# buq2/camera_calibrator

Hardware: AMD Instinct MI355X
Metric: LM residuals/sec (2*N_obs per LM iteration), single-camera intrinsics BA (higher is better)
Workload: dtype f64; 1 GPU; BASELINE.json configs[2]: single-camera intrinsics, 1000 frames x 500 pts per GPU, radial-tangential distortion, Zhang init, reference solver options (calibrator.cpp:314-321); frames_total=1000, points_per_frame=500, observations_total=500000, parallelism=frame-sharded x1, exchange=none

## Files before the change

camera_calibrator_amd/csrc/cc_device.hpp:

```cpp
#pragma once
#include "cc_common.hpp"

namespace cc {

typedef double d4 __attribute__((ext_vector_type(4)));
typedef double d2 __attribute__((ext_vector_type(2)));

constexpr int kStageDoublesPerWave = 64 * 16;

__device__ __forceinline__ int tri(int i, int j) { return i * (i + 1) / 2 + j; }

template <int CTRL>
__device__ __forceinline__ double dpp_f64(double v) {
  const int lo = __builtin_amdgcn_update_dpp(0, __double2loint(v), CTRL, 0xf, 0xf, false);
  const int hi = __builtin_amdgcn_update_dpp(0, __double2hiint(v), CTRL, 0xf, 0xf, false);
  return __hiloint2double(hi, lo);
}
__device__ __forceinline__ double row_pair_sum(double v) {
  const auto l = __builtin_amdgcn_permlane16_swap((unsigned)__double2loint(v), (unsigned)__double2loint(v), false, false);
  const auto h = __builtin_amdgcn_permlane16_swap((unsigned)__double2hiint(v), (unsigned)__double2hiint(v), false, false);
  return __hiloint2double((int)h[0], (int)l[0]) + __hiloint2double((int)h[1], (int)l[1]);
}
__device__ __forceinline__ double half_pair_sum(double v) {
  const auto l = __builtin_amdgcn_permlane32_swap((unsigned)__double2loint(v), (unsigned)__double2loint(v), false, false);
  const auto h = __builtin_amdgcn_permlane32_swap((unsigned)__double2hiint(v), (unsigned)__double2hiint(v), false, false);
  return __hiloint2double((int)h[0], (int)l[0]) + __hiloint2double((int)h[1], (int)l[1]);
}
template <int LOG2 = 0>
__device__ __forceinline__ double wave_sum_mod(double v) {
  static_assert(LOG2 >= 0 && LOG2 <= 3, "strides 1, 2, 4, 8");
  if (LOG2 == 0) v += dpp_f64<0xB1>(v);
  if (LOG2 <= 1) v += dpp_f64<0x4E>(v);
  if (LOG2 <= 2) v += dpp_f64<0x124>(v);
  v += dpp_f64<0x128>(v);
  return half_pair_sum(row_pair_sum(v));
}
__device__ __forceinline__ double wave_sum(double v) { return wave_sum_mod<0>(v); }
__device__ __forceinline__ double row16_sum(double v) {
  v += dpp_f64<0xB1>(v);
  v += dpp_f64<0x4E>(v);
  v += dpp_f64<0x141>(v);
  v += dpp_f64<0x140>(v);
  return v;
}
__device__ __forceinline__ double row16_max(double v) {
  v = fmax(v, dpp_f64<0xB1>(v));
  v = fmax(v, dpp_f64<0x4E>(v));
  v = fmax(v, dpp_f64<0x141>(v));
  v = fmax(v, dpp_f64<0x140>(v));
  return v;
}

__device__ __forceinline__ double lane_bcast(double v, int l) {
  return __hiloint2double(__builtin_amdgcn_readlane(__double2hiint(v), l), __builtin_amdgcn_readlane(__double2loint(v), l));
}

template <int S>
__device__ __forceinline__ bool chol_solve_rows(double (&a)[S], double b, double (&x)[S]) {
  bool ok = true;
  double inv[S];
#pragma unroll
  for (int j = 0; j < S; ++j) {
    const double d = lane_bcast(a[j], j);
    ok = ok && (d > 0.0) && isfinite(d);
    const double r = rsqrt(d);
    inv[j] = r;
    a[j] *= r;
#pragma unroll
    for (int k = j + 1; k < S; ++k) a[k] = fma(-a[j], lane_bcast(a[j], k), a[k]);
  }
#pragma unroll
  for (int j = 0; j < S; ++j) {
    const double y = lane_bcast(b, j) * inv[j];
    x[j] = y;
    b = fma(-a[j], y, b);
  }
#pragma unroll
  for (int i = S - 1; i >= 0; --i) {
    double acc = x[i];
#pragma unroll
    for (int k = i + 1; k < S; ++k) acc = fma(-lane_bcast(a[i], k), x[k], acc);
    x[i] = acc * inv[i];
  }
  return ok;
}

__device__ __forceinline__ void lds_barrier() { asm volatile("s_waitcnt lgkmcnt(0)\n\ts_barrier" ::: "memory"); }

__device__ __forceinline__ void wave_lds_fence() { __builtin_amdgcn_fence(__ATOMIC_ACQ_REL, "wavefront"); }

__device__ __forceinline__ void stage_row(double* stage, int lane, const double* v) {
#pragma unroll
  for (int j = 0; j < 8; ++j) {
    d2 val;
    val.x = v[2 * j];
    val.y = v[2 * j + 1];
    *reinterpret_cast<d2*>(&stage[lane * 16 + ((j ^ (lane & 7)) << 1)]) = val;
  }
}

__device__ __forceinline__ void gram_rows(const double* stage, int lane, d4& acc0, d4& acc1) {
  const int c = lane & 15, sub = lane >> 4;
#pragma unroll
  for (int m = 0; m < 16; m += 2) {
    const int r0 = 4 * m + sub, r1 = 4 * (m + 1) + sub;
    const double a0 = stage[r0 * 16 + (((c >> 1) ^ (r0 & 7)) << 1) + (c & 1)];
    const double a1 = stage[r1 * 16 + (((c >> 1) ^ (r1 & 7)) << 1) + (c & 1)];
    acc0 = __builtin_amdgcn_mfma_f64_16x16x4f64(a0, a0, acc0, 0, 0, 0);
    acc1 = __builtin_amdgcn_mfma_f64_16x16x4f64(a1, a1, acc1, 0, 0, 0);
  }
}

__device__ __forceinline__ void gram_operands(const double* stage, int lane, double* a) {
  const int c = lane & 15, sub = lane >> 4;
#pragma unroll
  for (int m = 0; m < 16; ++m) {
    const int r = 4 * m + sub;
    a[m] = stage[r * 16 + (((c >> 1) ^ (r & 7)) << 1) + (c & 1)];
  }
}

__device__ __forceinline__ void gram_products(const double* a, d4& acc0, d4& acc1) {
#pragma unroll
  for (int m = 0; m < 16; m += 2) {
    acc0 = __builtin_amdgcn_mfma_f64_16x16x4f64(a[m], a[m], acc0, 0, 0, 0);
    acc1 = __builtin_amdgcn_mfma_f64_16x16x4f64(a[m + 1], a[m + 1], acc1, 0, 0, 0);
  }
}

__device__ __forceinline__ void gram_rows_ahead(const double* stage, int lane, d4& acc0, d4& acc1) {
  double a[16];
  gram_operands(stage, lane, a);
  __builtin_amdgcn_sched_barrier(0);
  gram_products(a, acc0, acc1);
  __builtin_amdgcn_sched_barrier(0);
}



__device__ __forceinline__ int p2p_slot(const P2pDev& X, int kind, unsigned long long epoch, int rank) {
  const int base = kind == 0 ? 0 : 2 * kP2pMaxRanks * X.sw[0];
  return base + ((int)(epoch & 1ull) * kP2pMaxRanks + rank) * X.sw[kind];
}

__device__ inline void p2p_post(const P2pDev& X, int kind, unsigned long long epoch, int rank, int nranks,
                                const double* src, int n, int first = 0) {
  const int off = p2p_slot(X, kind, epoch, rank) + 2 * first;
  const unsigned long long tag = (epoch & 0xffffffffull) << 32;
  const int words = 2 * n;
  for (int idx = threadIdx.x; idx < words * nranks; idx += blockDim.x) {
    const int r = idx / words, w = idx - r * words;
    const unsigned long long bits = (unsigned long long)__double_as_longlong(src[w >> 1]);
    const unsigned long long half = (w & 1) ? (bits >> 32) : (bits & 0xffffffffull);
    __hip_atomic_store(X.box[r] + off + w, tag | half, __ATOMIC_RELAXED, __HIP_MEMORY_SCOPE_SYSTEM);
  }
}

__device__ __forceinline__ double p2p_poll_sum(const P2pDev& X, int kind, unsigned long long epoch, int rank, int nranks,
                                               int i, long long t0, int* s_ok) {
  const unsigned long long tag = epoch & 0xffffffffull;
  const unsigned long long* base = X.box[rank] + 2 * i;
  unsigned long long lo[kP2pMaxRanks], hi[kP2pMaxRanks];
  for (;;) {
    bool all = true;
#pragma unroll
    for (int r = 0; r < kP2pMaxRanks; ++r) {
      if (r < nranks) {
        const unsigned long long* p = base + p2p_slot(X, kind, epoch, r);
        lo[r] = __hip_atomic_load(p, __ATOMIC_RELAXED, __HIP_MEMORY_SCOPE_SYSTEM);
        hi[r] = __hip_atomic_load(p + 1, __ATOMIC_RELAXED, __HIP_MEMORY_SCOPE_SYSTEM);
      }
    }
#pragma unroll
    for (int r = 0; r < kP2pMaxRanks; ++r)
      if (r < nranks) all = all && (lo[r] >> 32) == tag && (hi[r] >> 32) == tag;
    if (all) break;
    if (wall_clock64() - t0 > kP2pTimeoutTicks) { *s_ok = 0; break; }
    __builtin_amdgcn_s_sleep(1);
  }
  double a = 0.0;
#pragma unroll
  for (int r = 0; r < kP2pMaxRanks; ++r)
    if (r < nranks) {
      const double v = __longlong_as_double((long long)((hi[r] << 32) | (lo[r] & 0xffffffffull)));
      a = r == 0 ? v : a + v;
    }
  return a;
}

__device__ inline double p2p_collect(const P2pDev& X, int kind, unsigned long long epoch, int rank, int nranks,
                                     int n, int* s_ok) {
  if (threadIdx.x == 0) *s_ok = 1;
  __syncthreads();
  double a = 0.0;
  if ((int)threadIdx.x < n) a = p2p_poll_sum(X, kind, epoch, rank, nranks, threadIdx.x, wall_clock64(), s_ok);
  __syncthreads();
  return a;
}

__device__ inline void p2p_collect_to(const P2pDev& X, int kind, unsigned long long epoch, int rank, int nranks,
                                      int n, double* dst, int* s_ok) {
  if (threadIdx.x == 0) *s_ok = 1;
  __syncthreads();
  const long long t0 = wall_clock64();
  for (int i = threadIdx.x; i < n; i += blockDim.x) dst[i] = p2p_poll_sum(X, kind, epoch, rank, nranks, i, t0, s_ok);
  __syncthreads();
}

}
```

camera_calibrator_amd/csrc/cc_intrinsics_persist.hip:

```cpp
#include "cc_intrinsics_persist.hpp"
#include "cc_persist_dev.hpp"
#include "cc_persist_pack.hpp"
#include "cc_persist_publish.hpp"
#include "cc_persist_sum.hpp"

namespace cc {


constexpr int persist_lds_doubles(int teams) { return teams * 4 * kStageDoublesPerWave + teams * 2 * 256 + teams * 192 + 512; }

enum { TM_Y = 0, TM_POSE = 60, TM_SP = 76, TM_STEP = 84, TM_R = 100, TM_T = 109, TM_KC = 112, TM_STEP2 = 122, TM_XN2 = 123,
       TM_QW = 124, TM_STAT = 128  };
enum { WG_INTR = 0 , WG_X = 64 , WG_DS = 66 ,
       WG_SS = 80 , WG_R0 = 96 ,
       WG_RO = 97 , WG_OPT = 100 ,
       WG_TAB = 104 ,
       WG_TGI = 416 , WG_TZ = 456  };

static_assert(TM_POSE - TM_Y >= 6 * 10 && TM_SP - TM_POSE >= 2 * 8 && TM_STEP - TM_SP >= 6 && TM_R - TM_STEP >= 15 && TM_T - TM_R >= 9 && TM_KC - TM_T >= 3 &&
              TM_STEP2 - TM_KC >= 9 && TM_QW - TM_XN2 >= 1 && TM_STAT - TM_QW >= 4 && TM_STAT + 4 + 9 <= 192,
              "per-team scratch: Y (6 x 10), two poses, pose scale, step (9 + 6), R, t, intrinsics, scalars, statistics row -- inside the 192 doubles persist_lds_doubles gives a team");
static_assert(WG_X - WG_INTR >= 2 * 16 && WG_DS - WG_X >= 2 && WG_SS - WG_DS >= 9 && WG_R0 - WG_SS >= 9 && WG_RO - WG_R0 >= 1 && WG_OPT - WG_RO >= 1 && WG_TAB - WG_OPT >= 4 &&
              WG_TZ - WG_TGI >= 80 / 2 && WG_TZ + 80 / 2 <= 512,
              "workgroup scratch: both intrinsics, broadcast (2 + 9), scales, options, tables of the 80-slot row -- inside the 512 doubles of persist_lds_doubles");

template <int NC, int NG, int BATCH = 8>
__device__ __forceinline__ void gather_rows(const u64* box, int G, unsigned tag, int ncols, int maxcol, double* s_part,
                                            double* out, unsigned* fail, int* s_ok, int tshift) {
  const int tid = threadIdx.x, col = tid % NC, grp = tid / NC;
  if (tid == 0) *s_ok = 1;
  __syncthreads();
  if (grp < NG && col < ncols) {
    double acc = 0.0;
    bool good = true;
    const long long t0 = wall_clock64();
    for (int r0 = grp; r0 < G && good; r0 += BATCH * NG) {
      u64 lo[BATCH], hi[BATCH];
      for (unsigned spins = 0;; ++spins) {
#pragma unroll
        for (int u = 0; u < BATCH; ++u) {
          const int r = r0 + u * NG;
          const u64* p = box + (size_t)(r < G ? r : r0) * (2 * NC) + 2 * col;
          lo[u] = ag_ld(p);
          hi[u] = ag_ld(p + 1);
        }
        bool ok = true;
#pragma unroll
        for (int u = 0; u < BATCH; ++u) ok = ok && (unsigned)(lo[u] >> 32) == tag && (unsigned)(hi[u] >> 32) == tag;
        if (ok) break;
        if ((spins & 63u) == 63u && (timed_out(t0, tshift) || ag_ld32(fail) != 0u)) { good = false; break; }
        __builtin_amdgcn_s_sleep(1);
      }
      if (!good) break;
#pragma unroll
      for (int u = 0; u < BATCH; ++u) {
        if (r0 + u * NG < G) {
          const double v = ungranule(lo[u], hi[u]);
          acc = col == maxcol ? fmax(acc, v) : acc + v;
        }
      }
    }
    s_part[grp * NC + col] = acc;
    if (!good) *s_ok = 0;
  }
  __syncthreads();
  if (tid < ncols) {
    double a = 0.0;
    if (tid == maxcol) { for (int g = 0; g < NG; ++g) a = fmax(a, s_part[g * NC + tid]); }
    else { for (int g = 0; g < NG; ++g) a += s_part[g * NC + tid]; }
    out[tid] = a;
  }
  __syncthreads();
}

template <int THREADS>
__device__ __forceinline__ void gather_stats4(const u64* box, int G, unsigned tag, double* s_part, double* out, unsigned* fail, int* s_ok, int tshift) {
  constexpr int RPT = 1024 / THREADS;
  static_assert(THREADS / 4 * RPT == kPMaxWorkers, "one statistics row per four threads: the host caps the worker grid at kPMaxWorkers");
  const int tid = threadIdx.x, col = tid & 3, lane = tid & 63, wave = tid >> 6;
  if (tid == 0) *s_ok = 1;
  __syncthreads();
  u64 lo[RPT], hi[RPT];
  bool good = true;
  const long long t0 = wall_clock64();
  for (unsigned spins = 0;; ++spins) {
    bool ok = true;
#pragma unroll
    for (int k = 0; k < RPT; ++k) {
      const int r = (tid >> 2) + k * (THREADS / 4);
      const u64* p = box + (size_t)(r < G ? r : 0) * (2 * kPStatCols) + 2 * col;
      lo[k] = ag_ld(p);
      hi[k] = ag_ld(p + 1);
    }
#pragma unroll
    for (int k = 0; k < RPT; ++k) ok = ok && (unsigned)(lo[k] >> 32) == tag && (unsigned)(hi[k] >> 32) == tag;
    if (ok) break;
    if ((spins & 63u) == 63u && (timed_out(t0, tshift) || ag_ld32(fail) != 0u)) { good = false; break; }
    __builtin_amdgcn_s_sleep(1);
  }
  double acc = 0.0;
#pragma unroll
  for (int k = 0; k < RPT; ++k)
    if ((tid >> 2) + k * (THREADS / 4) < G) acc += ungranule(lo[k], hi[k]);
  acc = wave_sum_mod<2>(acc);
  if (lane < 4) s_part[wave * 4 + lane] = acc;
  if (!good) *s_ok = 0;
  __syncthreads();
  if (tid < 4) {
    double a = 0.0;
#pragma unroll
    for (int w = 0; w < THREADS / 64; ++w) a += s_part[w * 4 + tid];
    out[tid] = a;
  }
  __syncthreads();
}

__device__ __forceinline__ size_t persist_box_word(int c, int g, int G) {
  return kPBoxColumnMajor ? ((size_t)c * (size_t)G + (size_t)g) * 2 : ((size_t)g * kPartialCols + (size_t)c) * 2;
}

template <int NG>
__device__ __forceinline__ void own_columns(const u64* box, u64* obox, int G, int w, unsigned tag, double* vals, unsigned* fail, int tid0, int tshift) {
  constexpr int kPer = (kPMaxWorkers + 63) / 64;
  int lane = tid0 & 63;
  asm volatile("" : "+v"(lane));
  asm volatile("" : "+s"(G));
  const int nc = (kPartialCols - 1 - w) / G + 1, items = nc * G, nL = persist_sum_groups(G);
  const u64* p[kPer];
#pragma unroll
  for (int u = 0; u < kPer; ++u) {
    const int i = lane + 64 * u, ic = i < items ? i : 0, k = ic / G;
    p[u] = box + persist_box_word(w + k * G, ic - k * G, G);
  }
  int gv[2], gn[2], gm[2];
#pragma unroll
  for (int u = 0; u < 2; ++u) {
    const int t = lane + 64 * u, tc = t < nc * nL ? t : 0, k = tc / nL, j = tc - k * nL;
    gv[u] = k * G + j * kPSumRows;
    gn[u] = persist_sum_group_rows(G, j);
    gm[u] = w + k * G == PC_GMAXP;
  }
  asm volatile("" : "+v"(gv[0]), "+v"(gv[1]), "+v"(gn[0]), "+v"(gn[1]), "+v"(gm[0]), "+v"(gm[1]));
  u64 lo[kPer], hi[kPer];
  bool good = true;
  const long long t0 = wall_clock64();
  for (unsigned spins = 0;; ++spins) {
#pragma unroll
    for (int u = 0; u < kPer; ++u) {
      lo[u] = ag_ld(p[u]);
      hi[u] = ag_ld(p[u] + 1);
    }
    bool ok = true;
#pragma unroll
    for (int u = 0; u < kPer; ++u) ok = ok && (unsigned)(lo[u] >> 32) == tag && (unsigned)(hi[u] >> 32) == tag;
    if (ok) break;
    if ((spins & 63u) == 63u && (timed_out(t0, tshift) || ag_ld32(fail) != 0u)) { good = false; break; }
    __builtin_amdgcn_s_sleep(1);
  }
  if (__any(!good)) {
    if (lane == 0) __hip_atomic_store(fail, 1u, __ATOMIC_RELAXED, __HIP_MEMORY_SCOPE_AGENT);
    return;
  }
#pragma unroll
  for (int u = 0; u < kPer; ++u)
    if (lane + 64 * u < items) vals[lane + 64 * u] = ungranule(lo[u], hi[u]);
  wave_lds_fence();
  double* Ls = vals + kPMaxWorkers + kPSumRows;
#pragma unroll
  for (int u = 0; u < 2; ++u)
    if (lane + 64 * u < nc * nL) Ls[lane + 64 * u] = persist_sum_group<NG>(vals + gv[u], gn[u], gm[u] != 0);
  wave_lds_fence();
  for (int k = lane; k < nc; k += 64) {
    const int c = w + k * G;
    const double total = persist_sum_group<NG>(Ls + k * nL, nL, c == PC_GMAXP);
    ag_st(obox + 2 * c, granule(tag, total, 0));
    ag_st(obox + 2 * c + 1, granule(tag, total, 1));
  }
}

__device__ __forceinline__ void gather_totals(const u64* box, unsigned tag, double* out, unsigned* fail, int* s_ok, int tshift) {
  const int tid = threadIdx.x;
  if (tid == 0) *s_ok = 1;
  __syncthreads();
  if (tid < kPartialCols) {
    const u64* p = box + 2 * tid;
    u64 lo, hi;
    bool good = true;
    const long long t0 = wall_clock64();
    for (unsigned spins = 0;; ++spins) {
      lo = ag_ld(p);
      hi = ag_ld(p + 1);
      if ((unsigned)(lo >> 32) == tag && (unsigned)(hi >> 32) == tag) break;
      if ((spins & 63u) == 63u && (timed_out(t0, tshift) || ag_ld32(fail) != 0u)) { good = false; break; }
      __builtin_amdgcn_s_sleep(1);
    }
    out[tid] = ungranule(lo, hi);
    if (!good) *s_ok = 0;
  }
  __syncthreads();
}

template <int THREADS>
__device__ __forceinline__ void persist_control(const IntrDev& P, const PersistDev& Q, double* lds) {
  double* s_part = lds;
  double* sv = lds + 1024;
  double* s_tot = lds + 1152;
  double* s_bc = lds + 1168;
  double* s_intr = lds + 1184;
  double* s_ss = lds + 1216;
  LmCtl* s_ctl = reinterpret_cast<LmCtl*>(lds + 1232);
  LmOpts* s_opts = reinterpret_cast<LmOpts*>(lds + 1252);
  cc_iteration* s_log = reinterpret_cast<cc_iteration*>(lds + 1264);
  int* s_int = reinterpret_cast<int*>(lds + 1296);
  u64* s_seq = reinterpret_cast<u64*>(lds + 1300);
  double* s_ccprev = lds + 1301;
  const int tid = threadIdx.x, wave = tid >> 6;
  static_assert(sizeof(cc_iteration) <= 32 * 8, "log record scratch");
  if (tid < (int)(sizeof(LmCtl) / 8)) reinterpret_cast<double*>(s_ctl)[tid] = 0.0;
  if (tid >= 32 && tid < 32 + (int)(sizeof(LmOpts) / 8)) reinterpret_cast<u64*>(s_opts)[tid - 32] = reinterpret_cast<const u64*>(P.opts)[tid - 32];
  if (tid >= 64 && tid < 64 + 32) s_intr[tid - 64] = 0.0;
  if (tid == 48 && P.host_pub) *s_seq = *P.pub_seq + 1ull;
  __syncthreads();
  if (tid < 9) s_intr[tid] = (Q.restart ? P.init_intr : P.intr)[tid];
  if (tid == 0) { s_int[1] = 0; s_int[3] = 0; s_int[5] = 0; s_int[6] = 0; s_int[7] = 0; *s_ccprev = 0.0; }
  __syncthreads();
  const LmOpts& o = *s_opts;
  const uint32_t mask = P.mask;

  for (int round = 0; round < Q.max_rounds; ++round) {
    const unsigned e1 = Q.epoch0 + 3u * (unsigned)round + 1u, e2 = e1 + 1u, e3 = e1 + 2u;
    const bool phase0 = round == 0;
    if (phase0) gather_rows<kPStatCols, THREADS / kPStatCols>(Q.sbox, Q.G, e1, 13, -1, s_part, s_tot, Q.fail, s_int, (phase0 ? Q.first_shift : Q.timeout_shift));
    else gather_stats4<THREADS>(Q.sbox, Q.G, e1, s_part, s_tot, Q.fail, s_int, (phase0 ? Q.first_shift : Q.timeout_shift));
    if (P.x.on) {
      const bool need = phase0 || (s_ctl->cand_pending && s_ctl->step_valid);
      if (need) {
        if (tid >= 13 && tid < 16) s_tot[tid] = 0.0;
        __syncthreads();
        const unsigned long long epoch = P.x.seq[1] + 1ull;
        p2p_post(P.x, 1, epoch, P.rank, P.nranks, s_tot, 16);
        int* s_ok2 = s_int + 4;
        const double a = p2p_collect(P.x, 1, epoch, P.rank, P.nranks, 16, s_ok2);
        if (tid < 16) s_tot[tid] = a;
        if (tid == 0) { P.x.seq[1] = epoch; if (!*s_ok2) s_int[0] = 0; }
        __syncthreads();
      }
    }
    if (tid == 0) {
      LmCtl c = *s_ctl;
      const int len0 = c.log_len, prev_cur = c.cur & 1, was_valid = c.step_valid;
      const int ro_now = s_int[3];
      const double prev_radius = c.radius;
      const double* kc0 = s_intr + (c.cur ? 16 : 0);
      const double* kc1 = s_intr + (c.cur ? 0 : 16);
      if (!s_int[0]) {
        __hip_atomic_store(Q.fail, 1u, __ATOMIC_RELAXED, __HIP_MEMORY_SCOPE_AGENT);
        c.done = 1; c.term = CC_FAILURE_EXCHANGE;
      } else if (phase0) {
        double xn2 = s_tot[ST_XNORM2];
#pragma unroll
        for (int i = 0; i < 9; ++i) {
          const double ki = kc0[i];
          xn2 += ki * ki;
          s_ss[i] = o.jacobi_scaling ? 1.0 / (1.0 + sqrt(s_tot[4 + i])) : 1.0;
        }
        lm_init(c, o, s_tot[ST_COST], sqrt(xn2));
      } else if (c.cand_pending) {
        double step2 = s_tot[ST_STEP2], xn2 = s_tot[ST_XNORM2];
        if (c.step_valid) {
#pragma unroll
          for (int i = 0; i < 9; ++i) {
            const double kc = kc1[i], k0 = kc0[i];
            const double d = kc - k0;
            step2 += d * d;
            xn2 += kc * kc;
          }
        }
        lm_decide(c, o, s_log, s_tot[ST_COST], s_tot[ST_QMODEL], step2, xn2);
      }
      if (!c.done && round + 1 >= Q.max_rounds) { c.done = 1; c.term = CC_NO_CONVERGENCE; }
      *s_ctl = c;
      s_int[1] = c.log_len != len0;
      s_int[2] = phase0 ? (!c.done && c.radius == o.initial_radius)
                        : (!ro_now && was_valid && !c.done && (c.cur & 1) == (prev_cur ^ 1) && c.radius == persist_spec_radius(prev_radius, o.max_radius));
      const bool accepted = !phase0 && (c.cur & 1) != prev_cur;
      if (ro_now) {
        s_int[6]++;
        if (!c.done) {
          if (Q.final_sweep == 1) s_int[5] = 1;
          if (accepted) s_int[7]++;
        }
      }
      int pred = 0;
      if (!c.done && s_int[0] && Q.final_sweep != 0 && !s_int[5] && !P.x.on && (phase0 || accepted)) {
        const double cc_k = phase0 ? 0.0 : s_log->cost_change;
        pred = Q.final_sweep == 2 || c.iter + 1 >= o.max_iterations || persist_predicts_end(cc_k, *s_ccprev, o.function_tolerance, c.x_cost);
      }
      if (accepted) *s_ccprev = s_log->cost_change;
      s_int[3] = pred;
      s_bc[0] = (double)((c.done ? 1 : 0) | ((c.cur & 1) << 3));
      s_bc[1] = c.radius;
#pragma unroll
      for (int i = 0; i < 9; ++i) s_bc[2 + i] = 0.0;
    }
    __syncthreads();
    const bool hit = s_int[2] != 0;
    const int pred_flag = s_int[3] ? 32 : 0;
    if (s_ctl->done || !hit) {
      if (tid < 22) ag_st(Q.xbox + tid, granule(e2, s_bc[tid >> 1], tid & 1));
      if (s_ctl->done) break;
    }
    const unsigned erow = hit ? e2 : e3;
    gather_totals(Q.lbox, erow, sv, Q.fail, s_int, (phase0 ? Q.first_shift : Q.timeout_shift));
    if (P.x.on) {
      if (tid >= kPartialCols && tid < kVecSolve) sv[tid] = 0.0;
      __syncthreads();
      if (tid == 0) { sv[kPartialCols + P.rank] = sv[PC_GMAXP]; sv[PC_GMAXP] = 0.0; }
      __syncthreads();
      const unsigned long long epoch = P.x.seq[0] + 1ull;
      p2p_post(P.x, 0, epoch, P.rank, P.nranks, sv, kVecSolve);
      int* s_ok2 = s_int + 4;
      const double a = p2p_collect(P.x, 0, epoch, P.rank, P.nranks, kVecSolve, s_ok2);
      if (tid < kVecSolve) sv[tid] = a;
      if (tid == 0) { P.x.seq[0] = epoch; if (!*s_ok2) s_int[0] = 0; }
      __syncthreads();
      if (tid == 0) {
        double g = 0.0;
        for (int r = 0; r < P.nranks && r < 32; ++r) g = fmax(g, sv[kPartialCols + r]);
        sv[PC_GMAXP] = g;
      }
      __syncthreads();
    }
    if (wave == 0) {
      int lane = tid & 63;
      asm volatile("" : "+v"(lane));
      const int cur = s_ctl->cur & 1;
      const double radius = s_ctl->radius;
      const double gl = (lane < 9 && !((mask >> lane) & 1u)) ? fabs(sv[PC_GS + lane]) : sv[PC_GMAXP];
      const double k_l = s_intr[cur * 16 + (lane < 9 ? lane : 8)], ss_l = s_ss[lane < 9 ? lane : 8];
      bool ok = !(sv[PC_FAIL] > 0.0);
      double x[9];
      {
#pragma clang fp contract(off)
        const int i = lane < 9 ? lane : 8;
        const bool pin_i = (mask >> i) & 1u;
        const double si = s_ss[i];
        const double damp = clampd(sv[PC_HDIAG + i] * (si * si), o.min_lm_diagonal, o.max_lm_diagonal) / radius;
        double a[9];
#pragma unroll
        for (int k = 0; k < 9; ++k) {
          const int kk = k <= i ? k : i;
          const int idx = kk * 9 - kk * (kk - 1) / 2 + (i - kk);
          double v = sv[idx] * (s_ss[kk] * si);
          if (k == i) v += damp;
          const bool pin_k = (mask >> kk) & 1u;
          if (pin_i || pin_k) v = (k == i) ? 1.0 : 0.0;
          a[k] = v;
        }
        const double b = pin_i ? 0.0 : sv[PC_B + i] * si;
        ok = chol_solve_rows<9>(a, b, x) && ok;
#pragma unroll
        for (int j = 0; j < 9; ++j) ok = ok && isfinite(x[j]);
      }
      const double gmax = row16_max(gl);
      const bool go = s_int[0] && !(gmax <= o.gradient_tolerance) && !(radius < o.min_radius);
      if (lane < 9) {
        double xs = 0.0;
#pragma unroll
        for (int j = 0; j < 9; ++j) xs = lane == j ? x[j] : xs;
        const double ds = go ? -xs : 0.0;
        const double d = ((mask >> lane) & 1u) ? 0.0 : ds * ss_l;
        s_bc[2 + lane] = d;
        s_intr[(cur ^ 1) * 16 + lane] = k_l + d;
      }
      if (lane == 0) {
        s_bc[0] = (double)((go ? 0 : 1) | (go && ok ? 2 : 0) | (hit ? 4 : 0) | (cur << 3) | pred_flag);
        s_bc[1] = radius;
        s_bc[12] = gmax;
      }
      wave_lds_fence();
      if (lane < 22) ag_st(Q.xbox + lane, granule(erow, s_bc[lane >> 1], lane & 1));
    }
    if (tid == 0) {
      const double gmax = s_bc[12];
      const bool ok = ((int)s_bc[0] & 2) != 0;
      cc_iteration* e = s_int[1] ? s_log : nullptr;
      if (e && e->accepted) e->gradient_max_norm = gmax;
      if (!s_int[0]) { __hip_atomic_store(Q.fail, 1u, __ATOMIC_RELAXED, __HIP_MEMORY_SCOPE_AGENT); s_ctl->done = 1; s_ctl->term = CC_FAILURE_EXCHANGE; }
      else if (lm_finalize(*s_ctl, o, gmax)) { s_ctl->step_valid = ok ? 1 : 0; s_ctl->cand_pending = 1; }
      if (e && s_ctl->log_len <= P.log_cap && !s_ctl->done) P.log[s_ctl->log_len - 1] = *e;
    }
    __syncthreads();
    if (s_ctl->done) break;
  }
  if (wave != 0) return;
  int lane = threadIdx.x;
  asm volatile("" : "+v"(lane));
  wave_lds_fence();
  const unsigned failed = ag_ld32(Q.fail);
  constexpr int kLogWords = (int)(sizeof(cc_iteration) / 8);
  static_assert(sizeof(LmCtl) == kPubDoubles * 8 && sizeof(cc_iteration) % 8 == 0 && kLogWords <= 64 && kPubWords <= 64, "one word per lane");
  static_assert(offsetof(LmCtl, done) == 0 && offsetof(LmCtl, term) == 4, "lanes 0 and 1 hold done and term");
  unsigned half = reinterpret_cast<const unsigned*>(s_ctl)[lane < kPubWords ? lane : 0];
  const int done = s_ctl->done, log_len = s_ctl->log_len;
  const bool owes_record = s_int[1] && log_len <= P.log_cap;
  const double intr_l = s_intr[lane & 31];
  const u64 log_l = reinterpret_cast<const u64*>(s_log)[lane < kLogWords ? lane : 0];
  if (failed != 0u) half = lane == 0 ? 1u : lane == 1 ? (unsigned)CC_FAILURE_EXCHANGE : half;
  else if (!done) half = lane == 0 ? 1u : lane == 1 ? (unsigned)CC_NO_CONVERGENCE : half;
  if (P.host_pub) {
    const u64 seq = *s_seq;
    if (lane < kPubWords) __hip_atomic_store(P.host_pub + kPubTaggedAt + lane, publish_word(publish_tag(seq), half), __ATOMIC_RELAXED, __HIP_MEMORY_SCOPE_SYSTEM);
    if (lane == 0) {
      __hip_atomic_store(P.host_pub, seq, __ATOMIC_RELAXED, __HIP_MEMORY_SCOPE_SYSTEM);
      *P.pub_seq = seq;
    }
  }
  if (lane < kPubWords) {
    reinterpret_cast<unsigned*>(P.ctl)[lane] = half;
    reinterpret_cast<unsigned*>(P.ctl_next)[lane] = half;
  }
  if (lane < 32 && failed == 0u) P.intr[lane] = intr_l;
  if (owes_record && lane < kLogWords) reinterpret_cast<u64*>(P.log + (log_len - 1))[lane] = log_l;
  if (lane < 2) Q.fs_counts[lane] = (unsigned)s_int[6 + lane];
}

template <int TEAMS>
__global__ __launch_bounds__(TEAMS * 256, TEAMS) void k_intr_persist(IntrDev P, PersistDev Q) {
  constexpr int THREADS = TEAMS * 256;
  extern __shared__ __attribute__((aligned(16))) char smem_raw[];
  double* s_stage = reinterpret_cast<double*>(smem_raw);
  if ((int)blockIdx.x == Q.G) { persist_control<THREADS>(P, Q, s_stage); return; }
  double* s_G = s_stage + TEAMS * 4 * kStageDoublesPerWave;
  double* s_tm = s_G + TEAMS * 2 * 256;
  double* s_wg = s_tm + TEAMS * 192;
#define CC_FRESH_TID(name) int name = tid0; asm volatile("" : "+v"(name))
  const int tid0 = threadIdx.x, wave = __builtin_amdgcn_readfirstlane(tid0 >> 6), team = wave >> 2, twave = wave & 3;
  const int sbase = (team & 3) * 64;
  const int64_t f = (int64_t)blockIdx.x * TEAMS + team;
  const bool has_frame = f < P.F;
  double* sm = s_tm + team * 192;
  double* tstage = s_stage + team * 4 * kStageDoublesPerWave;
  double* s_blk = tstage;
  double* Zs = tstage + 1024;
  double* red = tstage + 1100;
  unsigned char* pj = reinterpret_cast<unsigned char*>(s_wg + WG_TAB);
  unsigned char* pk = pj + 48;
  const uint32_t mask = P.mask;

  {
  const int tid = tid0, ttid = tid0 & 255;
  if (has_frame && ttid < 8) {
    const double v = ttid < 7 ? (Q.restart ? P.init_pose : P.pose)[(size_t)f * 8 + ttid] : 0.0;
    sm[TM_POSE + ttid] = v;
    sm[TM_POSE + 8 + ttid] = v;
  }
  if (ttid >= 64 && ttid < 64 + 60) sm[TM_Y + ttid - 64] = 0.0;
  if (tid < 32) s_wg[WG_INTR + tid] = 0.0;
  if (tid == 32) {
    const LmOpts* o = P.opts;
    s_wg[WG_OPT] = o->jacobi_scaling ? 1.0 : 0.0;
    s_wg[WG_OPT + 1] = o->min_lm_diagonal;
    s_wg[WG_OPT + 2] = o->max_lm_diagonal;
    s_wg[WG_OPT + 3] = o->max_radius;
    s_wg[WG_R0] = o->initial_radius;
  }
  if (tid == 33) {
    int oo = 0;
    for (int j = 0; j < 9; ++j)
      for (int k = j; k < 9; ++k) { pj[oo] = (unsigned char)j; pk[oo] = (unsigned char)k; ++oo; }
  }
  if (tid == 34) {
    bool fits = true;
    for (int k = 0; k < TEAMS; ++k) {
      const int64_t fk = (int64_t)blockIdx.x * TEAMS + k;
      if (fk < P.F && P.off[fk + 1] - P.off[fk] > (int64_t)kPackMaxPasses * kSweepThreads) fits = false;
    }
    s_wg[WG_RO] = fits ? 1.0 : 0.0;
  }
  if (tid >= 64 && tid < 64 + 16) s_wg[WG_X + tid - 64] = 0.0;
  if (tid >= 80 && tid < 80 + 16) s_wg[WG_SS + tid - 80] = 1.0;
  __syncthreads();
  if (tid < 9) s_wg[WG_INTR + tid] = (Q.restart ? P.init_intr : P.intr)[tid];
  if (tid >= 128 && tid < 128 + kPartialCols) {
    const int o = tid - 128;
    int gi = 0, z = 0;
    if (o < 45) {
      const int j = pj[o], k = pk[o];
      gi = j * 16 + k; z = j | (k << 8) | (1 << 16);
    } else if (o < 54) {
      const int j = o - 45;
      gi = j * 16 + 15; z = j | (9 << 8) | (1 << 16);
    } else if (o < 63) {
      const int j = o - 54;
      gi = j * 17;
    } else if (o >= PC_GS && o < PC_GS + 9) {
      gi = (o - PC_GS) * 16 + 15;
    }
    reinterpret_cast<int*>(s_wg + WG_TGI)[o] = gi;
    reinterpret_cast<int*>(s_wg + WG_TZ)[o] = z;
  }
  }

  int64_t s0 = 0, s1 = 0;
  if (has_frame) { s0 = P.off[f]; s1 = P.off[f + 1]; }
  const float2* uv2 = reinterpret_cast<const float2*>(P.uv);
  const int64_t wrem = s1 - s0 - twave * 64;
  const int npass = wrem > 0 ? (int)((wrem + kSweepThreads - 1) / kSweepThreads) : 0;
  const int64_t safe0 = s0 < P.N ? s0 : 0;
  float2 nm;
  float nX0, nX1, nX2;
  {
    const int64_t first = s0 + (tid0 & 255);
    const int64_t firstc = first < s1 ? first : safe0;
    nm = uv2[firstc];
    nX0 = P.xyz[firstc * 3]; nX1 = P.xyz[firstc * 3 + 1]; nX2 = P.xyz[firstc * 3 + 2];
  }
  __syncthreads();

  int cur = 0;
  double radius = 1.0;
  bool step_valid = true, failed = false;
  bool ends_next = false;
  for (int round = 0; round < Q.max_rounds; ++round) {
    const unsigned e1 = Q.epoch0 + 3u * (unsigned)round + 1u, e2 = e1 + 1u, e3 = e1 + 2u;
    const bool phase0 = round == 0;
    const bool do_sweep = phase0 || step_valid;
    const int dst = phase0 ? cur : (cur ^ 1);
    const bool resid_only = ends_next && do_sweep && __builtin_amdgcn_readfirstlane((int)s_wg[WG_RO]) != 0;
    if (do_sweep) {
      CC_FRESH_TID(tid);
      const int ttid = tid & 255, lane = tid & 63;
      const double* ds = s_wg + WG_DS;
      const double* ss = s_wg + WG_SS;
      if (has_frame) {
        const int st = ttid - sbase;
        if (st >= 0 && st < 6) {
          const double* Yr = sm + TM_Y + st * 10;
          double a = Yr[9];
#pragma unroll
          for (int j = 0; j < 9; ++j) a += Yr[j] * ds[j];
          sm[TM_STEP + 9 + st] = phase0 ? 0.0 : -a * sm[TM_SP + st];
        } else if (st >= 8 && st < 17) {
          const int j = st - 8;
          const double d = (phase0 || (mask & (1u << j))) ? 0.0 : ds[j] * ss[j];
          sm[TM_STEP + j] = d;
          const double kc = s_wg[WG_INTR + cur * 16 + j] + d;
          sm[TM_KC + j] = kc;
          if (team == 0 && !phase0) s_wg[WG_INTR + dst * 16 + j] = kc;
        }
      }
      __syncthreads();
      if (has_frame && ttid == sbase) {
        double q[4], t[3], dp[6];
#pragma unroll
        for (int i = 0; i < 4; ++i) q[i] = sm[TM_POSE + cur * 8 + i];
#pragma unroll
        for (int i = 0; i < 3; ++i) t[i] = sm[TM_POSE + cur * 8 + 4 + i];
#pragma unroll
        for (int i = 0; i < 6; ++i) dp[i] = sm[TM_STEP + 9 + i];
        double step2 = 0.0;
        if (!phase0) {
          double qn[4];
          quat_plus_tab(q, dp, qn);
#pragma unroll
          for (int i = 0; i < 4; ++i) { const double d = qn[i] - q[i]; step2 += d * d; q[i] = qn[i]; }
#pragma unroll
          for (int i = 0; i < 3; ++i) { const double tn = t[i] + dp[3 + i]; const double d = tn - t[i]; step2 += d * d; t[i] = tn; }
#pragma unroll
          for (int i = 0; i < 4; ++i) sm[TM_POSE + dst * 8 + i] = q[i];
#pragma unroll
          for (int i = 0; i < 3; ++i) sm[TM_POSE + dst * 8 + 4 + i] = t[i];
        }
        double R[9];
        quat_to_R(q, R);
#pragma unroll
        for (int i = 0; i < 9; ++i) sm[TM_R + i] = R[i];
#pragma unroll
        for (int i = 0; i < 3; ++i) sm[TM_T + i] = t[i];
        sm[TM_STEP2] = step2;
        sm[TM_XN2] = q[0] * q[0] + q[1] * q[1] + q[2] * q[2] + q[3] * q[3] + t[0] * t[0] + t[1] * t[1] + t[2] * t[2];
      }
      __syncthreads();
      {
        double qterm = 0.0;
        if (has_frame && !phase0) {
          const int a = ttid >> 4, b = ttid & 15;
          const double g_old = s_G[(team * 2 + cur) * 256 + ttid];
          if (a < 15) qterm = b < 15 ? 0.5 * sm[TM_STEP + a] * g_old * sm[TM_STEP + b] : sm[TM_STEP + a] * g_old;
        }
        const double qw = wave_sum(qterm);
        if (lane == 0) sm[TM_QW + twave] = qw;
      }
    }
    auto full_sweep = [&](const bool with_stats) {
    d4 acc0, acc1;
    {
      CC_FRESH_TID(tid);
      const int ttid = tid & 255, lane = tid & 63;
      double R[9], tt[3], kk[9];
#pragma unroll
      for (int i = 0; i < 9; ++i) R[i] = rfl(sm[TM_R + i]);
#pragma unroll
      for (int i = 0; i < 3; ++i) tt[i] = rfl(sm[TM_T + i]);
#pragma unroll
      for (int i = 0; i < 9; ++i) kk[i] = rfl(sm[TM_KC + i]);
      double* stage = s_stage + wave * kStageDoublesPerWave;
      acc0 = d4{0.0, 0.0, 0.0, 0.0};
      acc1 = d4{0.0, 0.0, 0.0, 0.0};
      if (npass == 0) { nm = float2{0.f, 0.f}; nX0 = nX1 = nX2 = 0.f; }
      for (int p = 0; p < npass; ++p) {
        const int64_t idx = s0 + (int64_t)p * kSweepThreads + ttid;
        const bool valid = idx < s1;
        const float2 m = nm;
        const float X0 = nX0, X1 = nX1, X2 = nX2;
        {
          const int64_t nidx = p + 1 < npass ? idx + kSweepThreads : s0 + ttid;
          const int64_t ic = nidx < s1 ? nidx : safe0;
          nm = uv2[ic];
          nX0 = P.xyz[ic * 3]; nX1 = P.xyz[ic * 3 + 1]; nX2 = P.xyz[ic * 3 + 2];
        }
        ObsCommon oc;
        huber_obs_common<TEAMS == 1>(kk, R, tt, (double)X0, (double)X1, (double)X2, oc);
        double v[16], ru, rv;
        const double wrow = valid ? 1.0 : 0.0;
        huber_residuals(kk, oc, (double)m.x, (double)m.y, ru, rv);
        huber_row_u(kk, oc, ru, v, wrow);
        stage_row(stage, lane, v);
        wave_lds_fence();
        gram_rows_ahead(stage, lane, acc0, acc1);
        wave_lds_fence();
        huber_row_v(kk, oc, rv, v, wrow);
        stage_row(stage, lane, v);
        wave_lds_fence();
        gram_rows_ahead(stage, lane, acc0, acc1);
        wave_lds_fence();
      }
      __syncthreads();
    }
    {
      CC_FRESH_TID(tid);
      const int ttid = tid & 255, lane = tid & 63;
#pragma unroll
      for (int r = 0; r < 4; ++r) s_blk[twave * 256 + ((lane >> 4) + 4 * r) * 16 + (lane & 15)] = acc0[r] + acc1[r];
      __syncthreads();
      const double g = gram_entry_held(mask, ttid) ? 0.0 : (s_blk[ttid] + s_blk[256 + ttid]) + (s_blk[512 + ttid] + s_blk[768 + ttid]);
      s_G[(team * 2 + dst) * 256 + ttid] = g;
      if (with_stats && ttid == 255) {
        sm[TM_STAT + ST_COST] = 0.5 * g;
        sm[TM_STAT + ST_QMODEL] = (sm[TM_QW] + sm[TM_QW + 1]) + (sm[TM_QW + 2] + sm[TM_QW + 3]);
        sm[TM_STAT + ST_STEP2] = sm[TM_STEP2];
        sm[TM_STAT + ST_XNORM2] = sm[TM_XN2];
      }
      if (with_stats && phase0 && ttid < 9 * 17 && ttid % 17 == 0) sm[TM_STAT + 4 + ttid / 17] = g;
      __syncthreads();
    }
    };
    auto resid_sweep = [&]() {
    {
      CC_FRESH_TID(tid);
      const int ttid = tid & 255, lane = tid & 63;
      double R[9], tt[3], kk[9];
#pragma unroll
      for (int i = 0; i < 9; ++i) R[i] = rfl(sm[TM_R + i]);
#pragma unroll
      for (int i = 0; i < 3; ++i) tt[i] = rfl(sm[TM_T + i]);
#pragma unroll
      for (int i = 0; i < 9; ++i) kk[i] = rfl(sm[TM_KC + i]);
      for (int p = 0; p < npass; ++p) {
        const int64_t idx = s0 + (int64_t)p * kSweepThreads + ttid;
        const bool valid = idx < s1;
        const float2 m = nm;
        const float X0 = nX0, X1 = nX1, X2 = nX2;
        {
          const int64_t nidx = p + 1 < npass ? idx + kSweepThreads : s0 + ttid;
          const int64_t ic = nidx < s1 ? nidx : safe0;
          nm = uv2[ic];
          nX0 = P.xyz[ic * 3]; nX1 = P.xyz[ic * 3 + 1]; nX2 = P.xyz[ic * 3 + 2];
        }
        ObsCommon oc;
        huber_obs_common<TEAMS == 1>(kk, R, tt, (double)X0, (double)X1, (double)X2, oc);
        double ru, rv;
        huber_residuals(kk, oc, (double)m.x, (double)m.y, ru, rv);
        const double wrow = valid ? 1.0 : 0.0;
        tstage[pack_write_slot(twave, p, 0, lane)] = ru * wrow;
        tstage[pack_write_slot(twave, p, 1, lane)] = rv * wrow;
      }
      __syncthreads();
    }
    {
      CC_FRESH_TID(tid);
      const int lane = tid & 63;
      if (has_frame && twave == (team & 3)) {
        const int64_t n = s1 - s0, wr = n - (int64_t)(pack_read_chain(lane) >> 1) * 64;
        const int mine = pack_read_chain(lane) < kPackChains && wr > 0 ? pack_chain_steps((int)((wr + kSweepThreads - 1) / kSweepThreads)) : 0;
        const int steps = pack_chain_steps((int)((n + kSweepThreads - 1) / kSweepThreads));
        d4 acc = d4{0.0, 0.0, 0.0, 0.0};
        for (int s0_ = 0; s0_ < steps; s0_ += kPackStepsPerPass) {
          double a[kPackStepsPerPass];
#pragma unroll
          for (int u = 0; u < kPackStepsPerPass; ++u) {
            const double v = tstage[pack_read_slot(s0_ + u, lane)];
            a[u] = s0_ + u < mine ? v : 0.0;
          }
          __builtin_amdgcn_sched_barrier(0);
#pragma unroll
          for (int u = 0; u < kPackStepsPerPass; ++u) acc = __builtin_amdgcn_mfma_f64_16x16x4f64(a[u], a[u], acc, 0, 0, 0);
          __builtin_amdgcn_sched_barrier(0);
        }
        double c[4];
#pragma unroll
        for (int w = 0; w < 4; ++w)
          c[w] = lane_bcast(acc[pack_diag_reg(2 * w)], pack_diag_lane(2 * w)) + lane_bcast(acc[pack_diag_reg(2 * w + 1)], pack_diag_lane(2 * w + 1));
        const double g = (c[0] + c[1]) + (c[2] + c[3]);
        if (lane == 0) {
          sm[TM_STAT + ST_COST] = 0.5 * g;
          sm[TM_STAT + ST_QMODEL] = (sm[TM_QW] + sm[TM_QW + 1]) + (sm[TM_QW + 2] + sm[TM_QW + 3]);
          sm[TM_STAT + ST_STEP2] = sm[TM_STEP2];
          sm[TM_STAT + ST_XNORM2] = sm[TM_XN2];
        }
      }
      __syncthreads();
    }
    };
    if (do_sweep) {
      if (resid_only) resid_sweep();
      else full_sweep(true);
    }
    {
      CC_FRESH_TID(tid);
      const int ncols = phase0 ? 13 : 4;
      const int stid = tid - 128;
      if (stid >= 0 && stid < 2 * ncols) {
        const int c = stid >> 1;
        double a = 0.0;
        if (do_sweep) {
#pragma unroll
          for (int k = 0; k < TEAMS; ++k)
            if ((int64_t)blockIdx.x * TEAMS + k < P.F) a += s_tm[k * 192 + TM_STAT + c];
        }
        ag_st(Q.sbox + (size_t)blockIdx.x * (2 * kPStatCols) + stid, granule(e1, a, stid & 1));
      }
    }
    auto eliminate_and_post = [&](const int cur_e, const double radius_e, const bool first, u64* box, const unsigned tag) {
    CC_FRESH_TID(tid_e);
    if (has_frame && (tid_e & 255) >= sbase && (tid_e & 255) < sbase + 16) {
      const int l = (tid_e & 255) - sbase;
      const double* Gl = s_G + (team * 2 + cur_e) * 256;
      const double* ss = s_wg + WG_SS;
      const bool jac = s_wg[WG_OPT] != 0.0;
      const double mn = s_wg[WG_OPT + 1], mx = s_wg[WG_OPT + 2];
      const double inv_radius = 1.0 / radius_e;
      double s[6], L[21];
#pragma unroll
      for (int i = 0; i < 6; ++i)
#pragma unroll
        for (int j = 0; j <= i; ++j) L[tri(i, j)] = Gl[(9 + i) * 16 + 9 + j];
      if (first) {
#pragma unroll
        for (int i = 0; i < 6; ++i) s[i] = jac ? 1.0 / (1.0 + sqrt(L[tri(i, i)])) : 1.0;
        if (l < 6) {
          double sl = 0.0;
#pragma unroll
          for (int i = 0; i < 6; ++i) sl = l == i ? s[i] : sl;
          sm[TM_SP + l] = sl;
        }
      } else {
#pragma unroll
        for (int i = 0; i < 6; ++i) s[i] = sm[TM_SP + i];
      }
#pragma unroll
      for (int i = 0; i < 6; ++i)
#pragma unroll
        for (int j = 0; j <= i; ++j) L[tri(i, j)] = s[i] * L[tri(i, j)] * s[j];
#pragma unroll
      for (int i = 0; i < 6; ++i) L[tri(i, i)] += clampd(L[tri(i, i)], mn, mx) * inv_radius;
      bool ok = true;
      double Li[6];
#pragma unroll
      for (int j = 0; j < 6; ++j) {
        double d = L[tri(j, j)];
#pragma unroll
        for (int k = 0; k < j; ++k) d -= L[tri(j, k)] * L[tri(j, k)];
        ok = ok && (d > 0.0) && isfinite(d);
        const double inv = rsqrt_pos(d);
        L[tri(j, j)] = d * inv;
        Li[j] = inv;
#pragma unroll
        for (int i = j + 1; i < 6; ++i) {
          double a = L[tri(i, j)];
#pragma unroll
          for (int k = 0; k < j; ++k) a -= L[tri(i, k)] * L[tri(j, k)];
          L[tri(i, j)] = a * inv;
        }
      }
#pragma unroll
      for (int i = 0; i < 21; ++i) L[i] = rfl(L[i]);
#pragma unroll
      for (int i = 0; i < 6; ++i) { Li[i] = rfl(Li[i]); s[i] = rfl(s[i]); }
      if (l < 10) {
        const double sc = l < 9 ? ss[l] : 1.0;
        const int col = l < 9 ? l : 15;
        double w[6], z[6], y[6];
#pragma unroll
        for (int i = 0; i < 6; ++i) w[i] = Gl[(9 + i) * 16 + col];
#pragma unroll
        for (int i = 0; i < 6; ++i) {
          double a = s[i] * w[i] * sc;
#pragma unroll
          for (int k = 0; k < i; ++k) a -= L[tri(i, k)] * z[k];
          z[i] = a * Li[i];
        }
#pragma unroll
        for (int i = 5; i >= 0; --i) {
          double a = z[i];
#pragma unroll
          for (int k = i + 1; k < 6; ++k) a -= L[tri(k, i)] * y[k];
          y[i] = a * Li[i];
        }
#pragma unroll
        for (int i = 0; i < 6; ++i) {
          Zs[i * 10 + l] = z[i];
          sm[TM_Y + i * 10 + l] = y[i];
        }
      }
      if (l == 0) red[PC_FAIL] = ok ? 0.0 : 1.0;
    }
    if (has_frame && (tid_e & 255) >= sbase && (tid_e & 255) < sbase + 64) {
      const int l64 = (tid_e & 255) - sbase;
      const double* Gl = s_G + (team * 2 + cur_e) * 256;
      wave_lds_fence();
      const int* tgi = reinterpret_cast<const int*>(s_wg + WG_TGI);
      const int* tz = reinterpret_cast<const int*>(s_wg + WG_TZ);
      double accv[2];
      int zz_[2];
#pragma unroll
      for (int r = 0; r < 2; ++r) {
        const int o = l64 + 64 * r, oc = o < kPartialCols ? o : 0;
        zz_[r] = tz[oc];
        accv[r] = Gl[tgi[oc]];
      }
#pragma unroll
      for (int r = 0; r < 2; ++r) {
        const int zj = zz_[r] & 255, zk = (zz_[r] >> 8) & 255;
        double zz = 0.0;
#pragma unroll
        for (int i = 0; i < 6; ++i) zz += Zs[i * 10 + zj] * Zs[i * 10 + zk];
        const int o = l64 + 64 * r;
        const bool used = o < 63 || (o >= PC_GS && o < PC_GS + 9);
        if (o < kPartialCols && o != PC_FAIL && o != PC_GMAXP) red[o] = used ? accv[r] - ((zz_[r] >> 16) ? zz : 0.0) : 0.0;
      }
    }
    if (has_frame && (tid_e & 255) == (((team & 3) + 1) & 3) * 64) {
      const double* Gg = s_G + (team * 2 + cur_e) * 256;
      double q4[4], g6[6];
#pragma unroll
      for (int i = 0; i < 4; ++i) q4[i] = sm[TM_POSE + cur_e * 8 + i];
#pragma unroll
      for (int i = 0; i < 6; ++i) g6[i] = Gg[(9 + i) * 16 + 15];
      red[PC_GMAXP] = pose_grad_proj_max_tab(q4, g6);
    }
    __syncthreads();
    {
      CC_FRESH_TID(tid);
      if (tid < 2 * kPartialCols) {
        const int c = tid >> 1;
        double a = 0.0;
#pragma unroll
        for (int k = 0; k < TEAMS; ++k) {
          if ((int64_t)blockIdx.x * TEAMS + k < P.F) {
            const double v = s_stage[k * 4 * kStageDoublesPerWave + 1100 + c];
            a = c == PC_GMAXP ? fmax(a, v) : a + v;
          }
        }
        ag_st(box + persist_box_word(tid >> 1, (int)blockIdx.x, Q.G) + (tid & 1), granule(tag, a, tid & 1));
      }
    }
    if (wave == 3 && (int)blockIdx.x < kPartialCols)
      own_columns<THREADS / kPartialCols>(box, Q.lbox, Q.G, (int)blockIdx.x, tag, s_stage + 2048, Q.fail, tid_e, (phase0 ? Q.first_shift : Q.timeout_shift));
    };
    auto wait_bcast = [&](const unsigned tag) {
      CC_FRESH_TID(tid);
      if (wave == 0 && !bcast_wait(Q.xbox, tag, 11, s_wg + WG_X, Q.fail, tid & 63, (phase0 ? Q.first_shift : Q.timeout_shift))) {
        int gave_up = 17;
        asm volatile("" : "+s"(gave_up));
        s_wg[WG_X] = (double)gave_up;
      }
      __syncthreads();
    };

    const bool spec = do_sweep && !ends_next;
    const double radius_spec = phase0 ? s_wg[WG_R0] : persist_spec_radius(radius, s_wg[WG_OPT + 3]);
    if (spec) eliminate_and_post(dst, radius_spec, phase0, Q.pbox, e2);
    wait_bcast(e2);
    int fl = __builtin_amdgcn_readfirstlane((int)s_wg[WG_X]);
    if (fl & 16) failed = true;
    if (fl & 1) { cur = (fl >> 3) & 1; break; }
    if (fl & 4) {
      cur = dst;
      radius = rfl(radius_spec);
    } else {
      cur = (fl >> 3) & 1;
      radius = rfl(s_wg[WG_X + 1]);
      if (resid_only && cur == dst) full_sweep(false);
      eliminate_and_post(cur, radius, false, Q.rbox, e3);
      wait_bcast(e3);
      fl = __builtin_amdgcn_readfirstlane((int)s_wg[WG_X]);
      if (fl & 16) failed = true;
      if (fl & 1) { cur = (fl >> 3) & 1; break; }
    }
    step_valid = (fl & 2) != 0;
    ends_next = (fl & 32) != 0;
  }
  CC_FRESH_TID(tid_w);
  if (!failed && ag_ld32(Q.fail) == 0u && has_frame && (tid_w & 255) < 7) P.pose[((size_t)cur * P.F + f) * 8 + (tid_w & 255)] = sm[TM_POSE + cur * 8 + (tid_w & 255)];
  asm volatile("" ::"v"(nm.x), "v"(nX0), "v"(nX1), "v"(nX2));
}

template <int TEAMS>
static int resident_of(int device, int* out) {
  const int lds = persist_lds_doubles(TEAMS) * 8;
  CC_HIP(hipFuncSetAttribute(reinterpret_cast<const void*>(k_intr_persist<TEAMS>), hipFuncAttributeMaxDynamicSharedMemorySize, lds));
  int per_cu = 0, cus = 0;
  CC_HIP(hipOccupancyMaxActiveBlocksPerMultiprocessor(&per_cu, k_intr_persist<TEAMS>, TEAMS * 256, lds));
  CC_HIP(hipDeviceGetAttribute(&cus, hipDeviceAttributeMultiprocessorCount, device));
  *out = per_cu >= 1 ? cus : 0;
  return 0;
}

int persist_resident_workgroups(int device, int teams, int* out) {
  return teams == 1 ? resident_of<1>(device, out) : teams == 2 ? resident_of<2>(device, out) : resident_of<4>(device, out);
}

void persist_launch(const IntrDev& P, const PersistDev& Q, bool drop_control, hipStream_t stream) {
  const dim3 grid((unsigned)Q.G + (drop_control ? 0u : 1u));
  if (Q.teams == 1) hipLaunchKernelGGL(k_intr_persist<1>, grid, dim3(256), persist_lds_doubles(1) * 8, stream, P, Q);
  else if (Q.teams == 2) hipLaunchKernelGGL(k_intr_persist<2>, grid, dim3(512), persist_lds_doubles(2) * 8, stream, P, Q);
  else hipLaunchKernelGGL(k_intr_persist<4>, grid, dim3(1024), persist_lds_doubles(4) * 8, stream, P, Q);
}

}
```

Measured before the change: 35.55 billion residuals/s.

## Accumulate Gram matrix with 4x4 f64 MFMA blocks exploiting symmetry

Replaces the full 16x16x4 f64 MFMA Gram accumulation of staged Jacobian rows with a set of 4x4x4 f64 MFMA products covering only the needed diagonal and off-diagonal blocks. A new constexpr header defines the lane-to-block mapping, and the store step mirrors off-diagonal blocks into the symmetric half. The aim is to avoid redundant products in the symmetric normal-matrix build. In exchange it issues more, smaller MFMAs and more LDS operand loads per row pair, and the cross-lane bookkeeping is more complex.

```diff
diff --git a/camera_calibrator_amd/csrc/cc_device.hpp b/camera_calibrator_amd/csrc/cc_device.hpp
--- a/camera_calibrator_amd/csrc/cc_device.hpp
+++ b/camera_calibrator_amd/csrc/cc_device.hpp
@@ -1,5 +1,6 @@
 #pragma once
 #include "cc_common.hpp"
+#include "cc_gram_blocks.hpp"
 
 namespace cc {
 
@@ -134,6 +135,68 @@
   __builtin_amdgcn_sched_barrier(0);
   gram_products(a, acc0, acc1);
   __builtin_amdgcn_sched_barrier(0);
+}
+
+struct GramBlocks { double c[kGbProducts]; };
+constexpr int kGbBatchPairs = 2;
+
+__device__ __forceinline__ void gram_blocks_clear(GramBlocks& g) {
+#pragma unroll
+  for (int n = 0; n < kGbProducts; ++n) g.c[n] = 0.0;
+}
+template <int PAIR0, int NP>
+__device__ __forceinline__ void gram_block_operands(const double* stage, int lane, double* a) {
+  int base[kGbOperands];
+#pragma unroll
+  for (int o = 0; o < kGbOperands; ++o) {
+    const int r = gb_op_row(o, 0, lane), c = gb_op_comp(o, lane);
+    base[o] = r * 16 + (((c >> 1) ^ (r & 7)) << 1) + (c & 1);
+  }
+#pragma unroll
+  for (int p = 0; p < NP; ++p)
+#pragma unroll
+    for (int o = 0; o < kGbOperands; ++o) a[p * kGbOperands + o] = stage[base[o] + (PAIR0 + p) * kGbPairRows * 16];
+}
+template <int N>
+__device__ __forceinline__ void gram_block_product(const double* a, GramBlocks& g) {
+  g.c[N] = __builtin_amdgcn_mfma_f64_4x4x4f64(a[gb_prod_a(N)], a[gb_prod_b(N)], g.c[N], 0, 0, 0);
+}
+template <int NP>
+__device__ __forceinline__ void gram_block_products(const double* a, GramBlocks& g) {
+#pragma unroll
+  for (int p = 0; p < NP; ++p) {
+    gram_block_product<0>(a + p * kGbOperands, g);
+    gram_block_product<1>(a + p * kGbOperands, g);
+    gram_block_product<2>(a + p * kGbOperands, g);
+    gram_block_product<3>(a + p * kGbOperands, g);
+    gram_block_product<4>(a + p * kGbOperands, g);
+  }
+}
+template <int NP, int PAIR0 = 0>
+__device__ __forceinline__ void gram_blocks_ahead(const double* stage, int lane, GramBlocks& g) {
+  static_assert(kGbPairs % NP == 0, "whole batches");
+  if constexpr (PAIR0 < kGbPairs) {
+    double a[NP * kGbOperands];
+    gram_block_operands<PAIR0, NP>(stage, lane, a);
+    __builtin_amdgcn_sched_barrier(0);
+    gram_block_products<NP>(a, g);
+    __builtin_amdgcn_sched_barrier(0);
+    gram_blocks_ahead<NP, PAIR0 + NP>(stage, lane, g);
+  }
+}
+__device__ __forceinline__ void gram_blocks_store(const GramBlocks& g, int lane, double* blk) {
+  blk[gb_acc_row(0, lane) * 16 + gb_acc_col(0, lane)] = g.c[0] + g.c[1];
+  {
+    const double s = g.c[2] + g.c[3];
+    const int r = gb_acc_row(2, lane), c = gb_acc_col(2, lane);
+    blk[r * 16 + c] = s;
+    blk[c * 16 + r] = s;
+  }
+  {
+    const double s = g.c[4] + dpp_f64<0x128>(g.c[4]);
+    const int r = gb_acc_row(4, lane), c = gb_acc_col(4, lane);
+    blk[gb_store_mirrored(lane) ? c * 16 + r : r * 16 + c] = s;
+  }
 }
 
 
diff --git a/camera_calibrator_amd/csrc/cc_gram_blocks.hpp b/camera_calibrator_amd/csrc/cc_gram_blocks.hpp
--- /dev/null
+++ b/camera_calibrator_amd/csrc/cc_gram_blocks.hpp
@@ -0,0 +1,46 @@
+#pragma once
+
+#ifdef __HIPCC__
+#define CC_GB_FN __host__ __device__ constexpr
+#else
+#define CC_GB_FN constexpr
+#endif
+
+namespace cc {
+
+constexpr int kGbPairs = 8;
+constexpr int kGbPairRows = 8;
+constexpr int kGbOperands = 6;
+constexpr int kGbProducts = 5;
+enum { GB_A0 = 0, GB_A1 = 1, GB_R0 = 2, GB_R1 = 3, GB_Z = 4, GB_X = 5 };
+
+CC_GB_FN int gb_slot(int lane) { return (lane >> 2) & 3; }
+
+CC_GB_FN int gb_op_set(int o, int slot) { return o <= GB_R1 ? (o & 1) : slot >> 1; }
+CC_GB_FN int gb_op_group(int o, int slot) {
+  return o <= GB_A1 ? slot : o <= GB_R1 ? ((slot + 1) & 3) : o == GB_Z ? (slot & 1) : 2 + (slot & 1);
+}
+CC_GB_FN int gb_op_row(int o, int pair, int lane) { return 4 * (2 * pair + gb_op_set(o, gb_slot(lane))) + (lane >> 4); }
+CC_GB_FN int gb_op_comp(int o, int lane) { return 4 * gb_op_group(o, gb_slot(lane)) + (lane & 3); }
+
+CC_GB_FN int gb_prod_a(int n) { return n == 0 || n == 2 ? GB_A0 : n == 1 || n == 3 ? GB_A1 : GB_Z; }
+CC_GB_FN int gb_prod_b(int n) { return n == 0 ? GB_A0 : n == 1 ? GB_A1 : n == 2 ? GB_R0 : n == 3 ? GB_R1 : GB_X; }
+
+CC_GB_FN int gb_acc_chain(int n, int lane) { return gb_op_set(gb_prod_b(n), gb_slot(lane)); }
+CC_GB_FN int gb_acc_row(int n, int lane) { return 4 * gb_op_group(gb_prod_a(n), gb_slot(lane)) + (lane >> 4); }
+CC_GB_FN int gb_acc_col(int n, int lane) { return 4 * gb_op_group(gb_prod_b(n), gb_slot(lane)) + (lane & 3); }
+
+CC_GB_FN int gb_entry_src(int chain, int r, int c) {
+  for (int n = 0; n < kGbProducts; ++n)
+    for (int lane = 0; lane < 64; ++lane)
+      if (gb_acc_chain(n, lane) == chain && gb_acc_row(n, lane) == r && gb_acc_col(n, lane) == c) return n * 64 + lane;
+  return -1;
+}
+CC_GB_FN bool gb_entry_held(int chain, int r, int c) { return gb_entry_src(chain, r, c) >= 0; }
+CC_GB_FN int gb_entry_acc(int chain, int r, int c) { return (gb_entry_held(chain, r, c) ? gb_entry_src(chain, r, c) : gb_entry_src(chain, c, r)) >> 6; }
+CC_GB_FN int gb_entry_lane(int chain, int r, int c) { return (gb_entry_held(chain, r, c) ? gb_entry_src(chain, r, c) : gb_entry_src(chain, c, r)) & 63; }
+
+CC_GB_FN int gb_partner_lane(int lane) { return lane ^ 8; }
+CC_GB_FN bool gb_store_mirrored(int lane) { return gb_slot(lane) >= 2; }
+
+}
diff --git a/camera_calibrator_amd/csrc/cc_intrinsics_persist.hip b/camera_calibrator_amd/csrc/cc_intrinsics_persist.hip
--- a/camera_calibrator_amd/csrc/cc_intrinsics_persist.hip
+++ b/camera_calibrator_amd/csrc/cc_intrinsics_persist.hip
@@ -594,7 +594,7 @@
       }
     }
     auto full_sweep = [&](const bool with_stats) {
-    d4 acc0, acc1;
+    GramBlocks acc;
     {
       CC_FRESH_TID(tid);
       const int ttid = tid & 255, lane = tid & 63;
@@ -606,8 +606,7 @@
 #pragma unroll
       for (int i = 0; i < 9; ++i) kk[i] = rfl(sm[TM_KC + i]);
       double* stage = s_stage + wave * kStageDoublesPerWave;
-      acc0 = d4{0.0, 0.0, 0.0, 0.0};
-      acc1 = d4{0.0, 0.0, 0.0, 0.0};
+      gram_blocks_clear(acc);
       if (npass == 0) { nm = float2{0.f, 0.f}; nX0 = nX1 = nX2 = 0.f; }
       for (int p = 0; p < npass; ++p) {
         const int64_t idx = s0 + (int64_t)p * kSweepThreads + ttid;
@@ -628,12 +627,12 @@
         huber_row_u(kk, oc, ru, v, wrow);
         stage_row(stage, lane, v);
         wave_lds_fence();
-        gram_rows_ahead(stage, lane, acc0, acc1);
+        gram_blocks_ahead<kGbBatchPairs>(stage, lane, acc);
         wave_lds_fence();
         huber_row_v(kk, oc, rv, v, wrow);
         stage_row(stage, lane, v);
         wave_lds_fence();
-        gram_rows_ahead(stage, lane, acc0, acc1);
+        gram_blocks_ahead<kGbBatchPairs>(stage, lane, acc);
         wave_lds_fence();
       }
       __syncthreads();
@@ -641,8 +640,7 @@
     {
       CC_FRESH_TID(tid);
       const int ttid = tid & 255, lane = tid & 63;
-#pragma unroll
-      for (int r = 0; r < 4; ++r) s_blk[twave * 256 + ((lane >> 4) + 4 * r) * 16 + (lane & 15)] = acc0[r] + acc1[r];
+      gram_blocks_store(acc, lane, s_blk + twave * 256);
       __syncthreads();
       const double g = gram_entry_held(mask, ttid) ? 0.0 : (s_blk[ttid] + s_blk[256 + ttid]) + (s_blk[512 + ttid] + s_blk[768 + ttid]);
       s_G[(team * 2 + dst) * 256 + ttid] = g;
```

Result: faster. 37.53 billion residuals/s, median of 6 (+5.5%).
